# hiimmuc/SpeakerVerification

Measured on AMD Instinct MI355X. Metric: embeddings/sec (2 s @16 kHz), higher is better.
Workload: dtype bf16

## Files before the change

### speakerverification_amd/csrc/api.hip

```cpp
#include <algorithm>
#include <cstdlib>
#include <cstring>

#include "handle.h"

using namespace svhip;

namespace svhip {
RaggedCheckFn ecapa_ragged_check, rawnet2_ragged_check, rawnet3_ragged_check, conformer_ragged_check, titanet_ragged_check, resnetse_ragged_check;
RaggedEmbedFn ecapa_embed_ragged, rawnet2_embed_ragged, rawnet3_embed_ragged, conformer_embed_ragged, titanet_embed_ragged, resnetse_embed_ragged;
}

namespace {

thread_local std::string g_create_error;

enum DevOptParse { OPT_NO_ENV, OPT_SET, OPT_IS1, OPT_NUM };
struct DevOptRow { const char* name; int svhip_handle::DevOpts::*field; const char* env; DevOptParse parse; int dflt; };
#define SV_OPT(name, env, parse, dflt) {#name, &svhip_handle::DevOpts::name, env, parse, dflt}
const DevOptRow kDevOpts[] = {
    SV_OPT(layer_labels, "SVHIP_LAYER_LABELS", OPT_SET, 0),
    SV_OPT(x3_keep_f32, "SVHIP_X3_KEEP_F32", OPT_SET, 0),
    SV_OPT(r2_big, "SVHIP_R2_BIG", OPT_IS1, 0),
    SV_OPT(asp_v1, "SVHIP_ASP_V1", OPT_IS1, 0),
// ... 7 lines not shown
    SV_OPT(asnorm_norefit, nullptr, OPT_NO_ENV, 0),
    SV_OPT(rn_sinc_full, "SVHIP_RN_SINC_FULL", OPT_IS1, 0),
    SV_OPT(fbank32, "SVHIP_FBANK32", OPT_IS1, 0),
    SV_OPT(fbank_unfused, "SVHIP_FBANK_UNFUSED", OPT_IS1, 0),
    SV_OPT(pw3_cus, "SVHIP_PW3_CUS", OPT_NUM, -1),
    SV_OPT(pw3_tail_off, "SVHIP_PW3_TAIL_OFF", OPT_IS1, 0),
    SV_OPT(cv_off, "SVHIP_CV_OFF", OPT_IS1, 0),
    SV_OPT(n128_off, "SVHIP_N128_OFF", OPT_IS1, 0),
    SV_OPT(rn_pool_off, "SVHIP_RN_POOL_OFF", OPT_IS1, 0),
    SV_OPT(rn_step_off, "SVHIP_RN_STEP_OFF", OPT_IS1, 0),
    SV_OPT(rn_sinc_f32, "SVHIP_RN_SINC_F32", OPT_IS1, 0),
    SV_OPT(rn_tail_big, "SVHIP_RN_TAIL_BIG", OPT_IS1, 0),
    SV_OPT(r2_slices, "SVHIP_R2_SLICES", OPT_NUM, -1),
    SV_OPT(rn_conv_unfused, "SVHIP_RN_CONV_UNFUSED", OPT_IS1, 0),
    SV_OPT(rn_keep, "SVHIP_RN_KEEP", OPT_IS1, 0),
};
#undef SV_OPT

int none_check(const svhip_config& c, const char*& err) {
    if (c.compute == SVHIP_F16) { err = "SVHIP_F16 is RawNet2's 16-bit mode (ECAPA's is SVHIP_BF16)"; return SVHIP_ERR_UNSUPPORTED; }
    return SVHIP_OK;
}
int fbank_then_features(svhip_handle* h, const float* d_wav, int B);

const ModelOps kModels[] = {
    {SVHIP_MODEL_ECAPA,        ecapa_check,     ecapa_spec,     ecapa_finalize,     ecapa_alloc,     ecapa_embed_wave,    ecapa_forward,     ecapa_stage,     2,
     nullptr, ecapa_ragged_check, ecapa_embed_ragged},
    {SVHIP_MODEL_RAWNET2,      rawnet2_check,   rawnet2_spec,   rawnet2_finalize,   rawnet2_alloc,   rawnet2_forward,     nullptr,           rawnet2_stage,   4},
    {SVHIP_MODEL_RAWNET2_CONV, rawnet2_check,   rawnet2_spec,   rawnet2_finalize,   rawnet2_alloc,   rawnet2_forward,     nullptr,           rawnet2_stage,   4,
     nullptr, rawnet2_ragged_check, rawnet2_embed_ragged},
// ... 12 lines not shown
const ModelOps* model_ops(int model) {
    for (const ModelOps& m : kModels)
        if (m.model == model) return &m;
    return nullptr;
}

WeightSpec model_spec(const svhip_handle* h) {
    WeightSpec spec;
    if (const ModelOps* m = model_ops(h->cfg.model); m->spec) m->spec(h->cfg, spec);
    return spec;
}

int fbank_then_features(svhip_handle* h, const float* d_wav, int B) {
    int rc;
    if ((rc = run(h, "fbank", 0, [&]() { return launch_fbank(h->fb, d_wav, B, h->cfg.samples, h->T, h->d_feat, h->stream); }))) return rc;
    h->feat_is_stale = false;
    return model_ops(h->cfg.model)->embed_feat(h, h->d_feat, B);
}

}

namespace svhip {

hipEvent_t prof_event(svhip_handle* h) {
    if (!h->ev_free.empty()) { hipEvent_t e = h->ev_free.back(); h->ev_free.pop_back(); return e; }
    hipEvent_t e = nullptr;
    (void)hipEventCreate(&e);
    return e;
}

void prof_collect(svhip_handle* h) {
// ... 335 lines not shown
int svhip_embed_features(svhip_handle* h, const float* feat, int32_t B, int32_t T, float* emb_out, int32_t flags) {
    int rc = check_ready(h, B);
    if (rc) return rc;
    if (!feat || !emb_out) SV_FAIL(h, SVHIP_ERR_INVALID, "null pointer");
    const ModelOps* m = model_ops(h->cfg.model);
    if (!m->embed_feat) SV_FAIL(h, SVHIP_ERR_UNSUPPORTED, "embed_features needs a spectral model (ECAPA, TitaNet, Conformer, ResNetSE)");
    if (T != h->T) SV_FAIL(h, SVHIP_ERR_INVALID, "T=%d but the handle was created for T=%d frames", T, h->T);
    if ((flags & SVHIP_ASYNC) && (flags & (SVHIP_IN_DEVICE | SVHIP_OUT_DEVICE)) != (SVHIP_IN_DEVICE | SVHIP_OUT_DEVICE))
        SV_FAIL(h, SVHIP_ERR_INVALID, "SVHIP_ASYNC needs device pointers");
    SV_HIP(h, hipSetDevice(h->cfg.device));
    const float* d_in = feat;
    if (!(flags & SVHIP_IN_DEVICE)) {
        SV_HIP(h, hipMemcpyAsync(h->d_feat, feat, (size_t)B * h->cfg.n_mels * T * 4, hipMemcpyHostToDevice, h->stream));
        d_in = h->d_feat;
    }
    h->feat_is_stale = false;
    if ((rc = m->embed_feat(h, d_in, B))) return rc;
    if ((rc = emit_embeddings(h, B, emb_out, flags))) return rc;
    return finish(h, flags);
}

int svhip_embed_wave(svhip_handle* h, const float* wav, int32_t B, int32_t L, float* emb_out, int32_t flags) {
    int rc = check_ready(h, B);
    if (rc) return rc;
    if (!wav || !emb_out) SV_FAIL(h, SVHIP_ERR_INVALID, "null pointer");
    if (L != h->cfg.samples) SV_FAIL(h, SVHIP_ERR_INVALID, "L=%d but the handle was created for %d samples", L, h->cfg.samples);
    if ((flags & SVHIP_ASYNC) && (flags & (SVHIP_IN_DEVICE | SVHIP_OUT_DEVICE)) != (SVHIP_IN_DEVICE | SVHIP_OUT_DEVICE))
        SV_FAIL(h, SVHIP_ERR_INVALID, "SVHIP_ASYNC needs device pointers");
    const ModelOps* m = model_ops(h->cfg.model);
    if (!m->embed_wave) SV_FAIL(h, SVHIP_ERR_UNSUPPORTED, "model %d has no forward path in this build", h->cfg.model);
    SV_HIP(h, hipSetDevice(h->cfg.device));
// ... 139 lines not shown
    if (!rc && tmp) e = hipMemcpyAsync(wav_out, d_out, (size_t)B * L * 4, hipMemcpyDeviceToHost, h->stream);
    if (tmp || !(flags & SVHIP_ASYNC)) { const hipError_t e2 = hipStreamSynchronize(h->stream); if (e == hipSuccess) e = e2; }
    if (tmp) (void)hipFree(tmp);
    if (rc) return rc;
    SV_HIP(h, e);
    return SVHIP_OK;
}

int svhip_get_stage(svhip_handle* h, const char* name, float* out, int64_t* count) {
    if (!h || !name || !count) return SVHIP_ERR_INVALID;
    if (h->lastB <= 0) SV_FAIL(h, SVHIP_ERR_STATE, "no forward has run yet");
    const int B = h->lastB;
    const size_t rag_in = h->rag_levels ? (size_t)h->rag_rows[0] : 0;
    StageView v{nullptr, rag_in ? rag_in : (size_t)B * h->T, 0, 0, !h->bf16};
    const std::string n(name);
    if (n == "input" && h->X_in) { v.src = h->X_in; v.cols = v.ld = h->cfg.n_mels; }
    else if (n == "mel") {
        if (h->feat_is_stale) SV_FAIL(h, SVHIP_ERR_STATE, "stage mel: the last forward ran the fused front-end, which never forms the mel power "
                                      "tensor (option fbank_unfused = 1 keeps the separate kernels)");
        v.src = h->d_feat; v.rows = (size_t)B * h->cfg.n_mels; v.cols = v.ld = h->T; v.f32 = true;
        if (rag_in) { v.rows = 1; v.cols = v.ld = rag_in * h->cfg.n_mels; }
    }
    else {
        const ModelOps* m = model_ops(h->cfg.model);
        if (!m->stage) return unknown_stage(h, n);
        if (int rc = m->stage(h, n, out != nullptr, v)) return rc;
    }
    const size_t rows = v.rows, cols = v.cols;
    *count = (int64_t)(rows * cols);
    if (!out) return SVHIP_OK;
    SV_HIP(h, hipStreamSynchronize(h->stream));
// ... 63 lines not shown
```

### speakerverification_amd/csrc/api_ecapa.hip

```cpp
#include <algorithm>

#include "handle.h"

namespace svhip {

namespace {

struct EcapaState : ModelState {
    ConvLayer blocks0, mfa, asp_tdnn, asp_conv;
    ConvLayer tdnn1[3], tdnn2[3], res2[3][7];
    LinearLayer se1[3], se2[3], asp_ctx, fc;
    float* se2T[3] = {};
    void *se1_bf[3] = {}, *se2T_bf[3] = {};
    float *aspbn_scale = nullptr, *aspbn_shift = nullptr;

    bool xin_ready = false;
    bool x0_is_s32 = false;
    bool cat_f32_stale = false;
    bool h2_is_s32 = false;
    bool h1_split = false;
    void* cat_s32 = nullptr;
    void* h2_s32 = nullptr;
    void* u_s32[2] = {};
    void* X0 = nullptr;
    void *H1 = nullptr, *H2 = nullptr, *H3 = nullptr;
    void* CAT = nullptr;
    void* MFA = nullptr;
    void* ATT = nullptr;
    float* LOGITS = nullptr;
    float *d_mean = nullptr, *d_s1 = nullptr, *d_s2 = nullptr, *d_gstats = nullptr, *d_ctx = nullptr;
    float *d_pool_raw = nullptr, *d_pool_bn = nullptr;
// ... 117 lines not shown
    if ((rc = dev_alloc(h, &s.d_gstats, B * 2 * C3))) return rc;
    if ((rc = dev_alloc(h, &s.d_ctx, B * 128))) return rc;
    h->lin_part_per_utt = (size_t)((2 * C3 + 383) / 384) * (size_t)std::max(128, c.embed_dim);
    if ((rc = dev_alloc(h, &h->d_lin_part, B * h->lin_part_per_utt))) return rc;
    if ((rc = dev_alloc(h, &s.d_pool_raw, B * 2 * C3))) return rc;
    if ((rc = dev_alloc(h, &s.d_pool_bn, B * 2 * C3))) return rc;
    if (h->x3 && (rc = dev_alloc(h, reinterpret_cast<char**>(&h->s32_buf), M * C3 * 4 + 256))) return rc;
    if (h->x3 && C % 32 == 0 && (rc = dev_alloc(h, reinterpret_cast<char**>(&s.cat_s32), M * C3 * 4 + 256))) return rc;
    if (h->x3 && (C == 512 || C == 1024)) {
        if ((rc = dev_alloc(h, reinterpret_cast<char**>(&s.h2_s32), M * C * 4 + 256))) return rc;
        for (int i = 0; i < 2; ++i) if ((rc = dev_alloc(h, reinterpret_cast<char**>(&s.u_s32[i]), M * (C / 8) * 4 + 256))) return rc;
    }
    h->colsum_region = (int64_t)((M + 255) / 256 + 2) * 16 * C3;
    if ((rc = dev_alloc(h, &h->d_colsum, (size_t)4 * h->colsum_region))) return rc;
    return SVHIP_OK;
}

static int ecapa_forward_part(svhip_handle* h, const float* d_feat_all, int b0, int B) {
    auto& s = S(h);
    const svhip_config& c = h->cfg;
    const int T = h->T, M = B * T, C = c.channels, C3 = 3 * C, C8 = C / 8, e = h->esz;
    const bool bf = h->bf16;
    hipStream_t st = h->cur;
    const size_t r0 = (size_t)b0 * T;
    const float* d_feat = d_feat_all + (size_t)b0 * c.n_mels * T;
    void* X_in = off(h->X_in, r0 * c.n_mels, e);
    void* X0 = off(s.X0, r0 * C, e);
    void* H1 = off(s.H1, r0 * C, e);
    void* H2 = off(s.H2, r0 * C, e);
    void* H3 = off(s.H3, r0 * C, e);
// ... 36 lines not shown
    if (!s.xin_ready && (rc = run(h, "prologue", 0, [&]() {
             return launch_prologue(d_feat, X_in, bf, B, c.n_mels, T, c.log_input, h->in_w, h->in_b, d_pstats, st,
                                    h->x3 ? h->d_status : nullptr, h->host_flag_dev, (b0_cv && xscale) ? 3.0e38f : 65504.0f);
         }))) return rc;
    if (b0_cv) {
        const ConvLayer& L = s.blocks0;
        if (xscale && (rc = run(h, "in_scale", 0, [&]() {
                 return launch_in_scale(static_cast<const float*>(X_in), (int64_t)M * c.n_mels, reinterpret_cast<uint32_t*>(xscale + 4), xscale, st, L.cv_wscale);
             }))) return rc;
        if ((rc = run(h, "split_s32", 0, [&]() { return launch_split_s32(static_cast<const float*>(X_in), c.n_mels, h->s32_buf, M, L.cv_cin, st, L.cv_cin, c.n_mels, xscale); }))) return rc;
        if ((rc = run(h, "gemm_pw3cv", (double)M * L.flops_per_row, [&]() { return launch_gemm_pw3cv(q0, st); }))) return rc;
        b0_done = true;
        x0_s32 = q0.y_s32 != 0;
    }
    if (!b0_done) {
        GemmParams p = conv_params(h, s.blocks0, X_in, c.n_mels, X0, C, M, T);
        p.act1 = ACT_GELU;
        if ((rc = conv_gemm(h, s.blocks0, p))) return rc;
    }
    s.x0_is_s32 = x0_s32;
    const void* xin = x0_s32 ? nullptr : X0;
    int ldin = C;
    const void* xin32 = x0_s32 ? X0 : nullptr;
    int ldin32 = C;
    for (int i = 0; i < 3; ++i) {
        char* h2s = s.h2_s32 ? static_cast<char*>(s.h2_s32) + r0 * C * 4 : nullptr;
        char* us[2] = {s.u_s32[0] ? static_cast<char*>(s.u_s32[0]) + r0 * C8 * 4 : nullptr, s.u_s32[1] ? static_cast<char*>(s.u_s32[1]) + r0 * C8 * 4 : nullptr};
        auto step_params = [&](int j) {
            const ConvLayer& L = s.res2[i][j - 1];
            GemmParams q = conv_params(h, L, us[(j - 1) & 1], C8, h2s + (size_t)j * C8 * 4, C, M, T);
            q.W = L.Ws32; q.Wrows = L.N; q.x3 = 2; q.act1 = ACT_RELU;
            if (j < 7) { q.R = static_cast<const float*>(H1) + (size_t)(j + 1) * C8; q.ldr = C; q.Y2 = us[j & 1]; q.lda2 = C8; }
// ... 113 lines not shown
         }))) return rc;
    return SVHIP_OK;
}

int ecapa_forward(svhip_handle* h, const float* d_feat, int B) {
    S(h).cat_f32_stale = false;
    const bool two = h->lanes == 2 && B >= 64 && !h->x3;
    return forward_lanes(h, ecapa_forward_part, d_feat, B, two ? 2 : 1, (B / 2 + 3) & ~3);
}

int ecapa_embed_wave(svhip_handle* h, const float* d_wav, int B) {
    auto& s = S(h);
    const int L = h->cfg.samples, T = h->T;
    const bool fused = h->bf16 && !h->in_w && h->d_logmel && !h->opt.fbank_unfused && !h->opt.fbank32 && fbank_fused_supported(h->fb, L);
    int rc;
    if (fused) {
        if ((rc = run(h, "fbank_fused", 0, [&]() {
                 return launch_fbank_fused(h->fb, d_wav, B, L, T, h->cfg.log_input, h->d_logmel, h->d_fpart, h->X_in, h->stream);
             }))) return rc;
    } else if ((rc = run(h, "fbank", 0, [&]() { return launch_fbank(h->fb, d_wav, B, L, T, h->d_feat, h->stream); }))) return rc;
    s.xin_ready = fused;
    h->feat_is_stale = fused;
    rc = ecapa_forward(h, h->d_feat, B);
    s.xin_ready = false;
    return rc;
}

int ecapa_ragged_check(const svhip_config& c, const int32_t* lengths, int n, bool is_wave, std::string& err) {
    return rag_mel_check(c, lengths, n, is_wave, err, true, "hop_length / max_batch / samples", 5, " (block 3 reflect-pads 4 frames on each side)");
}

static void ecapa_rag_frames(const svhip_config& c, int64_t len, bool is_wave, int T[RAG_LEVELS]) { T[0] = (int)mel_frames(c, len, is_wave); }
static const RagRule kEcapaRag = {1, ecapa_rag_frames, true};

static int ecapa_forward_ragged(svhip_handle* h, const RagPack& pk) {
    auto& s = S(h);
    const svhip_config& c = h->cfg;
    const int C = c.channels, C3 = 3 * C, C8 = C / 8, e = h->esz;
    const bool bf = h->bf16;
// ... 120 lines not shown
```

### speakerverification_amd/csrc/api_gemm.hip

```cpp
#include "handle.h"

namespace svhip {

static const void* zero_page_for(const svhip_handle* h, const void* A) {
    const char* a = static_cast<const char*>(A);
    for (const TailedBuf& b : h->tailed)
        if (a >= b.base && a < b.base + b.bytes) return b.base + b.bytes;
    return h->d_zero;
}

GemmParams conv_params(const svhip_handle* h, const ConvLayer& L, const void* A, int lda, void* Y, int ldy, int M, int T) {
    GemmParams p;
    p.A = A; p.lda = lda; p.Y = Y; p.ldy = ldy;
    p.W = L.W; p.Wrows = L.Np; p.bias = L.bias; p.scale = L.scale; p.shift = L.shift;
    p.M = M; p.N = L.N; p.K = L.K; p.Kp = L.Kp; p.T = T; p.taps = L.taps; p.dil = L.dil; p.cin = L.cin;
    p.num_cu = h->num_cu; p.pw3_cus = h->opt.pw3_cus; p.tail_split = h->opt.pw3_tail_off ? 0 : 1;
    p.zeros = h->d_zeros; p.ones = h->d_ones; p.f16 = h->f16 ? 1 : 0;
    p.cv_off = h->opt.cv_off; p.n128_off = h->opt.n128_off;
    return p;
}

GemmPlan conv_plan(const svhip_handle* h, const ConvLayer& L, GemmParams p, const void* A_s32, int lda_s32) {
    GemmPlan g;
    p.zero_page = zero_page_for(h, p.A);
    const int M = p.M;
    const bool bf = h->bf16;
    g.flops = (double)M * (L.flops_per_row + 2.0 * L.N * p.K3);
    if (h->x3 && L.Ws32 && h->s32_buf && !p.A2 && !p.bias_utt && !p.out_f32 && !p.R) {
        GemmParams q = p;
        q.A = A_s32 ? A_s32 : h->s32_buf; q.lda = A_s32 ? lda_s32 : L.K; q.W = L.Ws32; q.x3 = 2;
        if (!gemm_pw3x3_supported(q)) q.side_a = q.side_b = nullptr, q.side_c = 0;
        if (!gemm_pw3x3_supported(q) && q.colsum) q.colsum = nullptr;
        if (gemm_pw3x3_supported(q)) {
// ... 40 lines not shown
```

### speakerverification_amd/csrc/api_ragged.hip

```cpp
#include <algorithm>
#include <cstdarg>

#include "handle.h"

namespace svhip {

int refuse(std::string& err, int code, const char* fmt, ...) {
    char b[512];
    va_list ap;
    va_start(ap, fmt);
    vsnprintf(b, sizeof(b), fmt, ap);
    va_end(ap);
    err = b;
    return code;
}

int rag_rows_fit(std::string& err, int i, int64_t rows, int64_t cap, const char* frames_name) {
    if (rows <= cap) return SVHIP_OK;
    return refuse(err, SVHIP_ERR_INVALID, "utterance %d: the pack reaches %lld frames, over the handle's capacity of max_batch * %s = %lld rows", i,
                  (long long)rows, frames_name, (long long)cap);
}

int rag_mel_check(const svhip_config& c, const int32_t* lengths, int n, bool is_wave, std::string& err, bool cfg_extra_ok, const char* cfg_names,
                  int min_frames, const char* why, RagUttRule* more, int64_t bound, int row_unit) {
// ... 38 lines not shown
    return SVHIP_OK;
}

RagTables::~RagTables() {
    for (auto& sl : slot) {
        if (sl.host) (void)hipHostFree(sl.host);
        if (sl.done) (void)hipEventDestroy(sl.done);
    }
}

static int rag_mel_input(svhip_handle* h, RagTables& rag, const float* in, bool in_host, bool is_wave, const int64_t* in_off, const int32_t* lengths,
                  int n, const int* mel0, int64_t* feat_off, const float** d_feat) {
    const svhip_config& c = h->cfg;
    int rc;
    *d_feat = h->d_feat;
    h->feat_is_stale = false;
    if (is_wave) {
        int64_t pos = 0;
        for (int u = 0; u < n; ++u) {
            const int L = lengths[u], T = mel0[u + 1] - mel0[u];
            const float* w = in + in_off[u];
            if (in_host) {
                SV_HIP(h, hipMemcpyAsync(rag.wav + pos, w, (size_t)L * 4, hipMemcpyHostToDevice, h->stream));
                w = rag.wav + pos;
                pos += L;
            }
            float* mel = h->d_feat + (size_t)mel0[u] * c.n_mels;
            if ((rc = run(h, "fbank", 0, [&]() { return launch_fbank(h->fb, w, 1, L, T, mel, h->stream); }))) return rc;
            feat_off[u] = (int64_t)mel0[u] * c.n_mels;
        }
    } else if (in_host) {
// ... 78 lines not shown
```

### speakerverification_amd/csrc/fbank.hip

```cpp
#include <stdlib.h>

#include "common.h"
#include "kernels.h"

namespace svhip {

namespace {

constexpr int FB_FRAMES = 32;
constexpr int FB_THREADS = 192;
constexpr int FB_PT_STRIDE = 289;
constexpr int FB_PAIRS_PER_WAVE = 3;

template <bool SPLIT>
__global__ __launch_bounds__(FB_THREADS) void fbank_kernel(FbankTables tb, const float* __restrict__ wav,
                                                           int L, int T, float* __restrict__ mel) {
    extern __shared__ __attribute__((aligned(16))) char smem[];
    const int ns = (FB_FRAMES - 1) * tb.hop + tb.win_length;
    const int ns_pad = ((ns + 15) & ~15) + 16;
    float* ys = reinterpret_cast<float*>(smem);
    float* pt = ys + ns_pad;
    float* melw = pt + FB_FRAMES * FB_PT_STRIDE;

    const int b = blockIdx.y;
// ... 655 lines not shown

bool fbank_fused_supported(const FbankTables& tb, int L) {
    return tb.sym_hi && tb.sym_lo && tb.n_fft == 512 && tb.win_length == 200 && tb.hop == 80 && tb.lpad == 156 && tb.mel_max_bin < 256 &&
           tb.n_mels % 4 == 0 && 32 * tb.n_mels <= 5 * FF_THREADS && tb.n_pairs >= 8 && L >= tb.n_fft && fbank_fused_lds(tb) <= 80 * 1024 &&
           (size_t)(32 * FF_PT_STRIDE + 32 * (tb.n_mels + 1)) * 4 <= (size_t)4 * FF_PLANE;
}

hipError_t launch_fbank_fused(const FbankTables& tb, const float* wav, int B, int L, int T, int log_input, float* logmel, float* partial,
                              void* out, hipStream_t stream) {
    if (!fbank_fused_supported(tb, L) || B <= 0) return hipErrorInvalidValue;
    const size_t lds = fbank_fused_lds(tb);
    static DeviceOnce attr;
    if (hipError_t e = set_max_dynamic_lds(attr, reinterpret_cast<const void*>(fbank_fused_kernel), 80 * 1024)) return e;
    const int ntiles = (T + FF_FRAMES - 1) / FF_FRAMES;
    hipLaunchKernelGGL(fbank_fused_kernel, dim3(ntiles, B), dim3(FF_THREADS), lds, stream, tb, wav, L, T, log_input, logmel, partial);
    hipLaunchKernelGGL(fbank_norm_kernel<bf16_t>, dim3((T + 63) / 64, B), dim3(256), 0, stream, logmel, partial, reinterpret_cast<bf16_t*>(out), T,
                       tb.n_mels, ntiles, log_input);
    return hipGetLastError();
}

hipError_t launch_prologue(const float* feat, void* out, bool out_bf16, int B, int n_mels, int T, int log_input,
                           const float* in_w, const float* in_b, float* stats, hipStream_t stream, uint32_t* status, uint32_t* host_flag, float limit) {
    const int rows = B * n_mels;
    hipLaunchKernelGGL(prologue_stats_kernel, dim3((rows + 3) / 4), dim3(256), 0, stream, feat, stats, rows, T,
                       log_input, in_w != nullptr ? 1 : 0);
    dim3 grid((T + 31) / 32, B);
    const size_t lds = (size_t)n_mels * 33 * sizeof(float);
    if (out_bf16)
        hipLaunchKernelGGL(prologue_apply_kernel<bf16_t>, grid, dim3(256), lds, stream, feat, stats,
                           reinterpret_cast<bf16_t*>(out), n_mels, T, log_input, in_w, in_b, status, host_flag, limit);
// ... 8 lines not shown
```

### speakerverification_amd/csrc/gemm_pw2.hip

```cpp
#include "common.h"
#include "kernels.h"
#include "gemm_epi.h"

namespace svhip {

namespace {

typedef __attribute__((address_space(3))) void lds_void;
typedef __attribute__((address_space(1))) const void gbl_void;

constexpr int QBM = 256, QBN = 256;
constexpr int HT = 16384;
constexpr int PW2_LDS = 8 * HT;
#ifdef QGROUP_M_OVERRIDE
constexpr int QGROUP_M = QGROUP_M_OVERRIDE;
#else
constexpr int QGROUP_M = 12;
#endif

#ifdef SVHIP_GEMM_DEBUG
constexpr bool DBG2 = true;
#else
constexpr bool DBG2 = false;
#endif
// ... 364 lines not shown
        if (p.lda3 <= 0 || p.lda % p.lda3 != 0 || ((p.lda / p.lda3) & (p.lda / p.lda3 - 1)) != 0 || p.lda3 % 8 != 0 || p.K3 > p.lda3) return false;
        if (reinterpret_cast<uintptr_t>(p.A3) & 15) return false;
    }
    if (p.taps > 1) {
        if (!p.zero_page || p.cin % 8 != 0 || p.taps * p.cin != p.K || p.T <= 0 || p.M % p.T != 0) return false;
        if (p.pad_mode == PAD_REFLECT && (p.taps / 2) * p.dil >= p.T) return false;
        if (p.Kp >= 65536 || p.cin > 1024) return false;
        return true;
    }
    return p.K == p.Kp;
}

hipError_t launch_gemm_pw2(const GemmParams& p, hipStream_t stream) {
    if (!gemm_pw2_supported(p, true) || p.M <= 0 || p.Wrows < p.N) return hipErrorInvalidValue;
    const bool conv = p.taps > 1;
    if (p.A3) return launch_inst<EPI_NONE, 2>(p, stream);
    if (p.act2 == ACT_LRELU03) return conv ? launch_inst<EPI_BN_LRELU03, 1>(p, stream) : launch_inst<EPI_BN_LRELU03, 0>(p, stream);
    switch (p.act1) {
        case ACT_NONE: return conv ? launch_inst<EPI_NONE, 1>(p, stream) : launch_inst<EPI_NONE, 0>(p, stream);
        case ACT_RELU: return conv ? launch_inst<EPI_RELU, 1>(p, stream) : launch_inst<EPI_RELU, 0>(p, stream);
        case ACT_GELU: return conv ? launch_inst<EPI_GELU, 1>(p, stream) : launch_inst<EPI_GELU, 0>(p, stream);
        case ACT_LRELU03: return conv ? launch_inst<EPI_LRELU03, 1>(p, stream) : launch_inst<EPI_LRELU03, 0>(p, stream);
        default: return hipErrorInvalidValue;
    }
}

}
```

### speakerverification_amd/csrc/handle.h

```cpp
#pragma once
#include "../../include/svhip.h"

#include <hip/hip_runtime.h>

#include <cstdio>
#include <initializer_list>
#include <map>
#include <memory>
#include <string>
#include <vector>

#include "common.h"
#include "kernels.h"

namespace svhip {

struct HostTensor {
    std::vector<float> data;
    std::vector<int64_t> shape;
    int64_t numel() const { int64_t n = 1; for (auto s : shape) n *= s; return n; }
};

struct ConvLayer {
    int N = 0, K = 0, Kp = 0, Np = 0, taps = 1, dil = 1, cin = 0;
// ... 47 lines not shown
        int score_tiled;
        int asnorm_norefit;
        int rn_sinc_full;
        int fbank32;
        int fbank_unfused;
        int pw3_cus;
        int pw3_tail_off;
        int cv_off;
        int n128_off;
        int rn_pool_off;
        int rn_step_off;
        int rn_sinc_f32;
        int rn_tail_big;
        int r2_slices;
        int rn_conv_unfused;
        int rn_keep;
    } opt;
    bool bf16 = false;
    bool f16 = false;
    int dt = svhip::DT_F32;
    bool x3 = false;
    bool finalized = false;
    std::string err;
    std::map<std::string, svhip::HostTensor> host_w;
    std::vector<void*> allocs;

    int T = 0;
    int esz = 4;

    svhip::FbankTables fb;
    int num_cu = 256;

    std::unique_ptr<svhip::ModelState> model;

    float* d_wav = nullptr;
    float* d_feat = nullptr;
    float* d_pstats = nullptr;
    float* d_xscale = nullptr;
    float* d_logmel = nullptr;
    float* d_fpart = nullptr;
    bool feat_is_stale = false;
    float* d_zero = nullptr;
    float *d_ones = nullptr, *d_zeros = nullptr;
    float* d_emb = nullptr;
    int lastB = 0;
    int64_t rag_rows[svhip::RAG_LEVELS] = {};
    int rag_levels = 0;
    void* X_in = nullptr;
    float *in_w = nullptr, *in_b = nullptr;
    float* d_colsum = nullptr;
    int64_t colsum_region = 0;
    float* d_lin_part = nullptr;
    size_t lin_part_per_utt = 0;
    void* s32_buf = nullptr;
    std::vector<svhip::TailedBuf> tailed;
    uint32_t* d_status = nullptr;
// ... 188 lines not shown
```

### speakerverification_amd/csrc/kernels.h

```cpp
#pragma once
#include <hip/hip_runtime.h>
#include <stdint.h>

#include <atomic>

#include "common.h"

namespace svhip {

struct DeviceOnce {
    std::atomic<uint64_t> mask{0};
    bool done(int dev) const { return dev >= 0 && dev < 64 && ((mask.load(std::memory_order_acquire) >> dev) & 1u); }
    void mark(int dev) { if (dev >= 0 && dev < 64) mask.fetch_or(1ull << dev, std::memory_order_release); }
};
inline hipError_t set_max_dynamic_lds(DeviceOnce& once, const void* fn, int bytes) {
    int dev = -1;
    hipError_t e = hipGetDevice(&dev);
    if (e != hipSuccess) return e;
    if (once.done(dev)) return hipSuccess;
    e = hipFuncSetAttribute(fn, hipFuncAttributeMaxDynamicSharedMemorySize, bytes);
    if (e == hipSuccess) once.mark(dev);
    return e;
}

// ... 13 lines not shown
    const float* ones = nullptr;
    const void* zero_page = nullptr;
    void* Y2 = nullptr;
    const void* R = nullptr;
    int ldr = 0;
    const void* A3 = nullptr;
    int lda3 = 0, K3 = 0;
    int y_s32 = 0;
    void* side_a = nullptr;
    void* side_b = nullptr;
    int side_lda = 0, side_ldb = 0, side_c = 0;
    int num_cu = 256;
    int n128_off = 0;
    int cv_off = 0;
    int pw3_cus = -1;
    const float* in_scale = nullptr;
    int tail_split = 1;
    void* ts = nullptr;
    int M = 0, N = 0, K = 0, Kp = 0;
    int lda = 0, lda2 = 0, ldy = 0, ld_bu = 0;
    int T = 1;
    uint32_t t_magic = 0;
    int taps = 1, dil = 1, cin = 0, pad_mode = 0;
    int act1 = 0, act2 = 0;
    int out_f32 = 0;
    int f16 = 0;
    int x3 = 0;
    int debug = 0;
    int Wrows = 0;
    const int* seg_off = nullptr;
// ... 6 lines not shown

constexpr int GEMM_BM = 128;
constexpr int GEMM_BN = 128;
constexpr int GEMM_BK_BYTES = 128;

inline int gemm_bk(bool bf16) { return bf16 ? 64 : 32; }
inline int round_up(int x, int m) { return (x + m - 1) / m * m; }

hipError_t launch_gemm(const GemmParams& p, bool bf16, hipStream_t stream);
enum GemmRoute : int { ROUTE_PW2 = 0, ROUTE_PW = 1, ROUTE_PW_NARROW = 2, ROUTE_GENERIC = 3, ROUTE_PW3 = 4, ROUTE_PW3CV = 5, ROUTE_N128 = 6 };
GemmRoute gemm_route(const GemmParams& p, bool bf16);
bool gemm_pw_supported(const GemmParams& p, bool bf16);
hipError_t launch_gemm_pw(const GemmParams& p, bool bf16, hipStream_t stream, bool narrow = false);
bool gemm_pw2_supported(const GemmParams& p, bool bf16);
hipError_t launch_gemm_pw2(const GemmParams& p, hipStream_t stream);
bool gemm_pw3_supported(const GemmParams& p, bool bf16);
hipError_t launch_gemm_pw3(const GemmParams& p, hipStream_t stream);
int pw3_grid_cap(const GemmParams& p);
bool gemm_pw3x3_supported(const GemmParams& p);
hipError_t launch_gemm_pw3x3(const GemmParams& p, hipStream_t stream);
bool r2_step_supported(const GemmParams& p);
hipError_t launch_r2_step(const GemmParams& p, hipStream_t stream);
bool rn_step_supported(const GemmParams& p, int mode);
hipError_t launch_rn_step(const GemmParams& p, int mode, hipStream_t stream);
bool gemm_pw3cv_supported(const GemmParams& p);
hipError_t launch_gemm_pw3cv(const GemmParams& p, hipStream_t stream);
bool gemm_n128_supported(const GemmParams& p);
hipError_t launch_gemm_n128(const GemmParams& p, hipStream_t stream);
bool gemm_pw3cv16_supported(const GemmParams& p);
hipError_t launch_gemm_pw3cv16(const GemmParams& p, hipStream_t stream);
// ... 50 lines not shown
    const int* mel_start = nullptr;
    const int* mel_len = nullptr;
    const int* mel_off = nullptr;
    int n_fft = 512, win_length = 200, hop = 80, n_mels = 80, n_bins = 257, lpad = 156;
    int n_pairs = 9;
    int n_q = 25;
    int mel_max_bin = 256;
    int force32 = 0;
    float preemph = 0.97f;
};
hipError_t launch_fbank(const FbankTables& tb, const float* wav, int B, int L, int T, float* mel, hipStream_t stream);

bool fbank_fused_supported(const FbankTables& tb, int L);
hipError_t launch_fbank_fused(const FbankTables& tb, const float* wav, int B, int L, int T, int log_input, float* logmel, float* partial,
                              void* out, hipStream_t stream);

hipError_t launch_prologue(const float* feat, void* out, bool out_bf16, int B, int n_mels, int T,
                           int log_input, const float* in_w, const float* in_b, float* stats, hipStream_t stream,
                           uint32_t* status = nullptr, uint32_t* host_flag = nullptr, float limit = 3.0e38f);

hipError_t launch_colmean(const void* X, int dt, int ldx, int B, int T, int C, float* mean, hipStream_t stream,
                          float* scratch = nullptr, int scratch_slices = 0);
hipError_t launch_colstats(const void* X, bool bf16, int ldx, int B, int T, int C, float* stats, float eps, hipStream_t stream);
size_t rowvec_linear_scratch_bytes(int B, int N, int K, bool short_rows = false);
hipError_t launch_rowvec_linear(const float* in, int ld_in, const float* W, const float* bias, float* out, int ld_out,
                                int B, int N, int K, int act, hipStream_t stream, float* part = nullptr, bool short_rows = false);
hipError_t launch_emb_out(const float* src, float* dst, int n, uint32_t* status, uint32_t* host_flag, hipStream_t stream);
hipError_t launch_se_mlp(const float* mean, const float* part, int T, const void* W1, const float* b1, const void* W2T,
                         const float* b2, float* s, bool w_bf16, int B, int C, int H, hipStream_t stream, int row_groups = 8);
hipError_t launch_se_apply(const void* h, int ldh, const float* s, const void* x, int ldx, void* out, int ldo,
// ... 258 lines not shown
```

Before: 59430.

## Fuse fbank mean-normalization into a weight-stationary blocks.0 conv kernel

Adds a new weight-stationary conv kernel for ECAPA's first 5-tap conv (80 input channels), which keeps the weights in registers and double-buffers reflect-padded input tiles in LDS. When the fused front-end is active, the kernel reads fp32 log-mel rows and per-utterance partial sums directly, subtracts the mean and casts to bf16 on the fly. This skips the separate fbank_norm kernel and the bf16 X_in round trip. The normalized input is now formed lazily only if a stage dump asks for it. The cost is a larger specialized code path with a heavier LDS footprint, and new state flags to track staleness.

```diff
diff --git a/speakerverification_amd/csrc/api.hip b/speakerverification_amd/csrc/api.hip
--- a/speakerverification_amd/csrc/api.hip
+++ b/speakerverification_amd/csrc/api.hip
@@ -45,6 +45,7 @@
     SV_OPT(r2_slices, "SVHIP_R2_SLICES", OPT_NUM, -1),
     SV_OPT(rn_conv_unfused, "SVHIP_RN_CONV_UNFUSED", OPT_IS1, 0),
     SV_OPT(rn_keep, "SVHIP_RN_KEEP", OPT_IS1, 0),
+    SV_OPT(b0_ws_off, "SVHIP_B0_WS_OFF", OPT_IS1, 0),
 };
 #undef SV_OPT
 
@@ -87,7 +88,7 @@
 int fbank_then_features(svhip_handle* h, const float* d_wav, int B) {
     int rc;
     if ((rc = run(h, "fbank", 0, [&]() { return launch_fbank(h->fb, d_wav, B, h->cfg.samples, h->T, h->d_feat, h->stream); }))) return rc;
-    h->feat_is_stale = false;
+    h->feat_is_stale = h->xin_is_stale = false;
     return model_ops(h->cfg.model)->embed_feat(h, h->d_feat, B);
 }
 
@@ -453,7 +454,7 @@
         SV_HIP(h, hipMemcpyAsync(h->d_feat, feat, (size_t)B * h->cfg.n_mels * T * 4, hipMemcpyHostToDevice, h->stream));
         d_in = h->d_feat;
     }
-    h->feat_is_stale = false;
+    h->feat_is_stale = h->xin_is_stale = false;
     if ((rc = m->embed_feat(h, d_in, B))) return rc;
     if ((rc = emit_embeddings(h, B, emb_out, flags))) return rc;
     return finish(h, flags);
@@ -623,7 +624,13 @@
     const size_t rag_in = h->rag_levels ? (size_t)h->rag_rows[0] : 0;
     StageView v{nullptr, rag_in ? rag_in : (size_t)B * h->T, 0, 0, !h->bf16};
     const std::string n(name);
-    if (n == "input" && h->X_in) { v.src = h->X_in; v.cols = v.ld = h->cfg.n_mels; }
+    if (n == "input" && h->X_in) {
+        v.src = h->X_in; v.cols = v.ld = h->cfg.n_mels;
+        if (h->xin_is_stale && out) {
+            SV_HIP(h, launch_fbank_norm(h->fb, h->d_logmel, h->d_fpart, h->X_in, B, h->T, h->cfg.log_input, h->stream));
+            h->xin_is_stale = false;
+        }
+    }
     else if (n == "mel") {
         if (h->feat_is_stale) SV_FAIL(h, SVHIP_ERR_STATE, "stage mel: the last forward ran the fused front-end, which never forms the mel power "
                                       "tensor (option fbank_unfused = 1 keeps the separate kernels)");
diff --git a/speakerverification_amd/csrc/api_ecapa.hip b/speakerverification_amd/csrc/api_ecapa.hip
--- a/speakerverification_amd/csrc/api_ecapa.hip
+++ b/speakerverification_amd/csrc/api_ecapa.hip
@@ -15,6 +15,7 @@
     float *aspbn_scale = nullptr, *aspbn_shift = nullptr;
 
     bool xin_ready = false;
+    bool xin_ws = false;
     bool x0_is_s32 = false;
     bool cat_f32_stale = false;
     bool h2_is_s32 = false;
@@ -162,6 +163,24 @@
     h->colsum_region = (int64_t)((M + 255) / 256 + 2) * 16 * C3;
     if ((rc = dev_alloc(h, &h->d_colsum, (size_t)4 * h->colsum_region))) return rc;
     return SVHIP_OK;
+}
+
+static GemmParams blocks0_params(svhip_handle* h, int b0, int B, bool from_logmel) {
+    auto& s = S(h);
+    const svhip_config& c = h->cfg;
+    const size_t r0 = (size_t)b0 * h->T;
+    GemmParams p = conv_params(h, s.blocks0, off(h->X_in, r0 * c.n_mels, h->esz), c.n_mels, off(s.X0, r0 * c.channels, h->esz), c.channels, B * h->T, h->T);
+    p.act1 = ACT_GELU;
+    if (from_logmel) {
+        p.ws_logmel = h->d_logmel + r0 * c.n_mels;
+        p.ws_fpart = h->d_fpart + (size_t)b0 * ((h->T + 63) / 64) * c.n_mels;
+        p.ws_sub_mean = c.log_input;
+    }
+    return p;
+}
+static bool blocks0_takes_ws(svhip_handle* h, const GemmParams& p) {
+    const GemmPlan g = conv_plan(h, S(h).blocks0, p);
+    return !g.x3 && g.route == ROUTE_PW2 && conv_ws_supported(g.q);
 }
 
 static int ecapa_forward_part(svhip_handle* h, const float* d_feat_all, int b0, int B) {
@@ -228,8 +247,9 @@
         x0_s32 = q0.y_s32 != 0;
     }
     if (!b0_done) {
-        GemmParams p = conv_params(h, s.blocks0, X_in, c.n_mels, X0, C, M, T);
-        p.act1 = ACT_GELU;
+        GemmParams p = blocks0_params(h, b0, B, s.xin_ws);
+        if (s.xin_ws && !blocks0_takes_ws(h, p))
+            SV_FAIL(h, SVHIP_ERR_STATE, "blocks.0 M%d: the front-end left only its fp32 rows and the kernel that reads them does not take this shape", M);
         if ((rc = conv_gemm(h, s.blocks0, p))) return rc;
     }
     s.x0_is_s32 = x0_s32;
@@ -373,15 +393,23 @@
     const int L = h->cfg.samples, T = h->T;
     const bool fused = h->bf16 && !h->in_w && h->d_logmel && !h->opt.fbank_unfused && !h->opt.fbank32 && fbank_fused_supported(h->fb, L);
     int rc;
+    bool ws = fused && !h->opt.b0_ws_off;
+    if (ws) {
+        const bool two = h->lanes == 2 && B >= 64;
+        const int per = two ? (B / 2 + 3) & ~3 : B;
+        for (int b0 = 0; b0 < B && ws; b0 += per) ws = blocks0_takes_ws(h, blocks0_params(h, b0, std::min(per, B - b0), true));
+    }
     if (fused) {
         if ((rc = run(h, "fbank_fused", 0, [&]() {
-                 return launch_fbank_fused(h->fb, d_wav, B, L, T, h->cfg.log_input, h->d_logmel, h->d_fpart, h->X_in, h->stream);
+                 return launch_fbank_fused(h->fb, d_wav, B, L, T, h->cfg.log_input, h->d_logmel, h->d_fpart, ws ? nullptr : h->X_in, h->stream);
              }))) return rc;
     } else if ((rc = run(h, "fbank", 0, [&]() { return launch_fbank(h->fb, d_wav, B, L, T, h->d_feat, h->stream); }))) return rc;
     s.xin_ready = fused;
+    s.xin_ws = ws;
     h->feat_is_stale = fused;
     rc = ecapa_forward(h, h->d_feat, B);
-    s.xin_ready = false;
+    s.xin_ready = s.xin_ws = false;
+    h->xin_is_stale = ws;
     return rc;
 }
 
diff --git a/speakerverification_amd/csrc/api_gemm.hip b/speakerverification_amd/csrc/api_gemm.hip
--- a/speakerverification_amd/csrc/api_gemm.hip
+++ b/speakerverification_amd/csrc/api_gemm.hip
@@ -16,7 +16,7 @@
     p.M = M; p.N = L.N; p.K = L.K; p.Kp = L.Kp; p.T = T; p.taps = L.taps; p.dil = L.dil; p.cin = L.cin;
     p.num_cu = h->num_cu; p.pw3_cus = h->opt.pw3_cus; p.tail_split = h->opt.pw3_tail_off ? 0 : 1;
     p.zeros = h->d_zeros; p.ones = h->d_ones; p.f16 = h->f16 ? 1 : 0;
-    p.cv_off = h->opt.cv_off; p.n128_off = h->opt.n128_off;
+    p.cv_off = h->opt.cv_off; p.n128_off = h->opt.n128_off; p.ws_off = h->opt.b0_ws_off;
     return p;
 }
 
diff --git a/speakerverification_amd/csrc/api_ragged.hip b/speakerverification_amd/csrc/api_ragged.hip
--- a/speakerverification_amd/csrc/api_ragged.hip
+++ b/speakerverification_amd/csrc/api_ragged.hip
@@ -76,7 +76,7 @@
     const svhip_config& c = h->cfg;
     int rc;
     *d_feat = h->d_feat;
-    h->feat_is_stale = false;
+    h->feat_is_stale = h->xin_is_stale = false;
     if (is_wave) {
         int64_t pos = 0;
         for (int u = 0; u < n; ++u) {
diff --git a/speakerverification_amd/csrc/conv_ws.hip b/speakerverification_amd/csrc/conv_ws.hip
--- /dev/null
+++ b/speakerverification_amd/csrc/conv_ws.hip
@@ -0,0 +1,278 @@
+#include <algorithm>
+
+#include "common.h"
+#include "kernels.h"
+#include "gemm_epi.h"
+
+namespace svhip {
+
+namespace {
+
+constexpr int WS_BM = 64;
+constexpr int WS_BN = 128;
+constexpr int WS_NCK = 13;
+constexpr int WS_TMIN = 32;
+constexpr int WS_SEGS = 3;
+constexpr int WS_MAXHALO = 2;
+constexpr int WS_CIN = 80;
+constexpr int WS_ROWS = WS_BM + 2 * WS_MAXHALO * WS_SEGS;
+constexpr int WS_OSTRIDE = 80;
+constexpr int WS_OPATCH = WS_BM * WS_OSTRIDE;
+constexpr int WS_THREADS = 256;
+constexpr int WS_NU = 16;
+#ifdef WS_ABL
+constexpr int ABL = WS_ABL;
+#else
+constexpr int ABL = 0;
+#endif
+
+struct WsGeom {
+    int rowb;
+    int ximg;
+    int mean_off;
+    int out_off;
+    int total;
+};
+__host__ __device__ constexpr WsGeom ws_geom(int cin) {
+    WsGeom g{};
+    g.rowb = cin * 2;
+    g.ximg = ((WS_ROWS + 1) * g.rowb + 63) & ~63;
+    g.mean_off = 2 * g.ximg;
+    g.out_off = g.mean_off + ((WS_NU * cin * 4 + 63) & ~63);
+    g.total = g.out_off + 4 * WS_OPATCH;
+    return g;
+}
+
+template <int MODE>
+__global__ __launch_bounds__(WS_THREADS, 2) void conv_ws_kernel(GemmParams p, int nslice, int G, int ntile) {
+    extern __shared__ __attribute__((aligned(16))) char smem[];
+    constexpr WsGeom g = ws_geom(WS_CIN);
+    constexpr int cin = WS_CIN;
+    const int tid = threadIdx.x, lane = tid & 63;
+    const int wave = __builtin_amdgcn_readfirstlane(tid >> 6);
+    const int r16 = lane & 15, q4 = lane >> 4;
+
+    const int id = blockIdx.x;
+    const int slice = (id >> 3) % nslice;
+    const int j = (id & 7) + 8 * ((id >> 3) / nslice);
+    if (j >= G) return;
+    const int tile_lo = (int)((int64_t)j * ntile / G), tile_hi = (int)((int64_t)(j + 1) * ntile / G);
+    if (tile_lo >= tile_hi) return;
+
+    const int T = p.T, halo = p.taps >> 1, TP = T + 2 * halo, B = p.M / T;
+    constexpr int cpr = cin >> 3;
+    constexpr int nchunk = WS_ROWS * cpr;
+    const int ntf = (T + 63) / 64;
+
+    const int nw0 = slice * WS_BN + wave * 32;
+    bf16x8 wf[2][WS_NCK];
+#pragma unroll
+    for (int jj = 0; jj < 2; ++jj) {
+        const char* wr = reinterpret_cast<const char*>(p.W) + ((int64_t)(nw0 + jj * 16 + r16) * p.Kp + q4 * 8) * 2;
+#pragma unroll
+        for (int c = 0; c < WS_NCK; ++c) wf[jj][c] = *reinterpret_cast<const bf16x8*>(wr + c * 64);
+    }
+    f32x4 b4[2], sc4[2], sh4[2];
+#pragma unroll
+    for (int jj = 0; jj < 2; ++jj) {
+        const int n = nw0 + jj * 16 + 4 * q4;
+        b4[jj] = p.bias ? *reinterpret_cast<const f32x4*>(p.bias + n) : f32x4{0.f, 0.f, 0.f, 0.f};
+        sc4[jj] = f32x4{1.f, 1.f, 1.f, 1.f}; sh4[jj] = f32x4{0.f, 0.f, 0.f, 0.f};
+        if (p.scale) { sc4[jj] = *reinterpret_cast<const f32x4*>(p.scale + n); sh4[jj] = *reinterpret_cast<const f32x4*>(p.shift + n); }
+    }
+
+    char* const ximg = smem;
+    float* const means = reinterpret_cast<float*>(smem + g.mean_off);
+    char* const opatch = smem + g.out_off + wave * WS_OPATCH;
+    const int ua = (tile_lo * WS_BM) / T;
+
+    constexpr int NIT = (nchunk + WS_THREADS - 1) / WS_THREADS;
+    u32x4 st[MODE == 0 ? NIT : 2 * NIT];
+    int st_r[NIT], st_cg[NIT];
+#pragma unroll
+    for (int it = 0; it < NIT; ++it) {
+        const int cc = min(it * WS_THREADS + tid, nchunk - 1);
+        st_r[it] = cc / cpr; st_cg[it] = cc - st_r[it] * cpr;
+    }
+    auto src_row = [&](int tile, int r, int& s) -> int64_t {
+        const int m0 = tile * WS_BM, u0 = m0 / T, t0 = m0 - u0 * T;
+        const int q = r + t0;
+        s = (q >= TP ? 1 : 0) + (q >= 2 * TP ? 1 : 0);
+        const int tr = reflect_idx(q - s * TP - halo, T);
+        return (int64_t)min(u0 + s, B - 1) * T + tr;
+    };
+    auto load_tile = [&](int tile) {
+#pragma unroll
+        for (int it = 0; it < NIT; ++it) {
+            int s;
+            const int64_t row = src_row(tile, st_r[it], s);
+            if (MODE == 0) {
+                st[it] = *reinterpret_cast<const u32x4*>(reinterpret_cast<const char*>(p.A) + (row * p.lda + st_cg[it] * 8) * 2);
+            } else {
+                const u32x4* src = reinterpret_cast<const u32x4*>(p.ws_logmel + row * cin + st_cg[it] * 8);
+                st[2 * it] = src[0]; st[2 * it + 1] = src[1];
+            }
+        }
+    };
+    auto store_tile = [&](int tile, char* img) {
+#pragma unroll
+        for (int it = 0; it < NIT; ++it) {
+            {
+                const int r = st_r[it], cg = st_cg[it];
+                u32x4 v;
+                if (MODE == 0) {
+                    v = st[it];
+                } else {
+                    const int m0 = tile * WS_BM, u0 = m0 / T, t0 = m0 - u0 * T, q = r + t0;
+                    const int s = (q >= TP ? 1 : 0) + (q >= 2 * TP ? 1 : 0);
+                    const float* mean = means + (min(u0 + s, B - 1) - ua) * cin + cg * 8;
+                    const f32x4 m_lo = *reinterpret_cast<const f32x4*>(mean);
+                    const f32x4 m_hi = *reinterpret_cast<const f32x4*>(mean + 4);
+                    const f32x4 a = __builtin_bit_cast(f32x4, st[2 * it]), b = __builtin_bit_cast(f32x4, st[2 * it + 1]);
+                    bf16x8 y;
+#pragma unroll
+                    for (int e = 0; e < 4; ++e) { y[e] = from_f32<bf16_t>(a[e] - m_lo[e]); y[4 + e] = from_f32<bf16_t>(b[e] - m_hi[e]); }
+                    v = __builtin_bit_cast(u32x4, y);
+                }
+                *reinterpret_cast<u32x4*>(img + r * g.rowb + cg * 16) = v;
+            }
+        }
+    };
+    load_tile(tile_lo);
+    if (MODE == 1) {
+        const int ub = min(B - 1, ((tile_hi - 1) * WS_BM) / T + WS_SEGS - 1);
+        const float rcin = 1.0f / (float)cin;
+        for (int idx = tid; idx < (ub - ua + 1) * cin; idx += WS_THREADS) {
+            const int du = (int)(((float)idx + 0.5f) * rcin), ch = idx - du * cin;
+            const float* src = p.ws_fpart + (int64_t)(ua + du) * ntf * cin + ch;
+            float sum = 0.0f;
+            for (int k0 = 0; k0 < ntf; k0 += 8) {
+                float v[8];
+#pragma unroll
+                for (int kk = 0; kk < 8; ++kk) v[kk] = src[min(k0 + kk, ntf - 1) * cin];
+#pragma unroll
+                for (int kk = 0; kk < 8; ++kk) sum = k0 + kk < ntf ? sum + v[kk] : sum;
+            }
+            means[idx] = p.ws_sub_mean ? sum / (float)T : 0.0f;
+        }
+        __syncthreads();
+    }
+    store_tile(tile_lo, ximg);
+    __syncthreads();
+
+    const int kmask = p.K - (WS_NCK - 1) * 32 - q4 * 8;
+    char* const Yb = reinterpret_cast<char*>(p.Y);
+    for (int tile = tile_lo; tile < tile_hi; ++tile) {
+        const int k = tile - tile_lo;
+        const char* xb = ximg + (k & 1) * g.ximg;
+        const int next = min(tile + 1, tile_hi - 1);
+        load_tile(next);
+        __builtin_amdgcn_sched_barrier(0);
+
+        const int m0 = tile * WS_BM, t0 = m0 - (m0 / T) * T;
+        int xo[4];
+#pragma unroll
+        for (int i = 0; i < 4; ++i) {
+            const int q = i * 16 + r16 + t0;
+            const int s = (q >= T ? 1 : 0) + (q >= 2 * T ? 1 : 0);
+            xo[i] = (i * 16 + r16 + 2 * halo * s) * g.rowb + q4 * 16;
+        }
+        f32x4 acc[4][2];
+#pragma unroll
+        for (int i = 0; i < 4; ++i) { acc[i][0] = b4[0]; acc[i][1] = b4[1]; }
+#pragma unroll
+        for (int c = 0; c < WS_NCK; ++c) {
+            bf16x8 xf[4];
+#pragma unroll
+            for (int i = 0; i < 4; ++i) {
+                xf[i] = *reinterpret_cast<const bf16x8*>(xb + xo[i] + c * 64);
+                if (c == WS_NCK - 1) {
+                    u32x4 z = __builtin_bit_cast(u32x4, xf[i]);
+                    z = kmask > 0 ? z : u32x4{0u, 0u, 0u, 0u};
+                    xf[i] = __builtin_bit_cast(bf16x8, z);
+                }
+            }
+#pragma unroll
+            for (int i = 0; i < 4; ++i)
+#pragma unroll
+                for (int jj = 0; jj < 2; ++jj)
+                    if (!(ABL & 1)) acc[i][jj] = Half16<bf16_t>::mfma16(wf[jj][c], xf[i], acc[i][jj]);
+        }
+
+        store_tile(next, ximg + ((k + 1) & 1) * g.ximg);
+
+#pragma unroll
+        for (int i = 0; i < 4; ++i)
+#pragma unroll
+            for (int jj = 0; jj < 2; ++jj) {
+                float v[4];
+                if (ABL & 4) { v[0] = acc[i][jj][0]; v[1] = acc[i][jj][1]; v[2] = acc[i][jj][2]; v[3] = acc[i][jj][3]; }
+                else act4<EPI_GELU>(v, acc[i][jj], sc4[jj], sh4[jj]);
+                typedef bf16_t bf16x4 __attribute__((ext_vector_type(4)));
+                const bf16x4 o = {static_cast<bf16_t>(v[0]), static_cast<bf16_t>(v[1]), static_cast<bf16_t>(v[2]), static_cast<bf16_t>(v[3])};
+                *reinterpret_cast<bf16x4*>(opatch + (i * 16 + r16) * WS_OSTRIDE + (jj * 16 + 4 * q4) * 2) = o;
+            }
+        __builtin_amdgcn_fence(__ATOMIC_RELEASE, "wavefront");
+        __builtin_amdgcn_wave_barrier();
+        __builtin_amdgcn_fence(__ATOMIC_ACQUIRE, "wavefront");
+#pragma unroll
+        for (int it = 0; it < 4; ++it) {
+            const int row = it * 16 + (lane >> 2), ch = lane & 3;
+            const u32x4 d = *reinterpret_cast<const u32x4*>(opatch + row * WS_OSTRIDE + ch * 16);
+            const int m = m0 + row;
+            if (m < p.M && !(ABL & 8)) *reinterpret_cast<u32x4*>(Yb + ((int64_t)m * p.ldy + nw0 + ch * 8) * 2) = d;
+        }
+        __syncthreads();
+    }
+}
+
+}
+
+static int ws_groups(const GemmParams& p) {
+    const int nslice = p.N / WS_BN, ntile = (p.M + WS_BM - 1) / WS_BM;
+    return std::max(1, std::min(ntile, 2 * p.num_cu / nslice));
+}
+static int ws_tiles_per_wg(const GemmParams& p) {
+    const int ntile = (p.M + WS_BM - 1) / WS_BM, G = ws_groups(p);
+    return (ntile + G - 1) / G;
+}
+
+bool conv_ws_supported(const GemmParams& p) {
+    if (p.ws_off || p.f16 || p.out_f32 || p.bias_utt || p.A2 || p.A3 || p.R || p.colsum || p.seg_off || p.rag_utt || p.x3) return false;
+    if (p.act1 != ACT_GELU || p.act2 != ACT_NONE || p.pad_mode != PAD_REFLECT || p.dil != 1) return false;
+    if (p.taps != 5 || p.cin != WS_CIN || p.taps * p.cin != p.K) return false;
+    if (p.K <= (WS_NCK - 1) * 32 || p.K > WS_NCK * 32 || p.Kp < WS_NCK * 32 || p.Kp % 8 != 0) return false;
+    if (p.T < WS_TMIN || p.M <= 0 || p.M % p.T != 0) return false;
+    if (p.N <= 0 || p.N % WS_BN != 0 || p.Wrows < p.N || p.ldy % 8 != 0 || p.ldy < p.N) return false;
+    if ((reinterpret_cast<uintptr_t>(p.W) | reinterpret_cast<uintptr_t>(p.Y)) & 15) return false;
+    if (p.bias && (reinterpret_cast<uintptr_t>(p.bias) & 15)) return false;
+    if (p.scale && (!p.shift || ((reinterpret_cast<uintptr_t>(p.scale) | reinterpret_cast<uintptr_t>(p.shift)) & 15))) return false;
+    if (p.ws_logmel) {
+        if (!p.ws_fpart || ((reinterpret_cast<uintptr_t>(p.ws_logmel) | reinterpret_cast<uintptr_t>(p.ws_fpart)) & 15)) return false;
+        if ((ws_tiles_per_wg(p) - 1) * WS_BM / p.T + WS_SEGS + 1 > WS_NU) return false;
+    } else if (!p.A || p.lda % 8 != 0 || p.lda < p.cin || (reinterpret_cast<uintptr_t>(p.A) & 15)) {
+        return false;
+    }
+    return true;
+}
+
+hipError_t launch_conv_ws(const GemmParams& p, hipStream_t stream) {
+    if (!conv_ws_supported(p)) return hipErrorInvalidValue;
+    const int nslice = p.N / WS_BN, ntile = (p.M + WS_BM - 1) / WS_BM;
+    const int G = ws_groups(p);
+    const int Gp = (G + 7) & ~7;
+    constexpr int lds = ws_geom(WS_CIN).total;
+    static_assert(lds <= 64 * 1024, "two workgroups per CU");
+    if (p.ws_logmel) {
+        static DeviceOnce attr;
+        if (hipError_t e = set_max_dynamic_lds(attr, reinterpret_cast<const void*>(conv_ws_kernel<1>), lds)) return e;
+        hipLaunchKernelGGL(conv_ws_kernel<1>, dim3(Gp * nslice), dim3(WS_THREADS), lds, stream, p, nslice, G, ntile);
+    } else {
+        static DeviceOnce attr;
+        if (hipError_t e = set_max_dynamic_lds(attr, reinterpret_cast<const void*>(conv_ws_kernel<0>), lds)) return e;
+        hipLaunchKernelGGL(conv_ws_kernel<0>, dim3(Gp * nslice), dim3(WS_THREADS), lds, stream, p, nslice, G, ntile);
+    }
+    return hipGetLastError();
+}
+
+}
diff --git a/speakerverification_amd/csrc/fbank.hip b/speakerverification_amd/csrc/fbank.hip
--- a/speakerverification_amd/csrc/fbank.hip
+++ b/speakerverification_amd/csrc/fbank.hip
@@ -693,6 +693,13 @@
     if (hipError_t e = set_max_dynamic_lds(attr, reinterpret_cast<const void*>(fbank_fused_kernel), 80 * 1024)) return e;
     const int ntiles = (T + FF_FRAMES - 1) / FF_FRAMES;
     hipLaunchKernelGGL(fbank_fused_kernel, dim3(ntiles, B), dim3(FF_THREADS), lds, stream, tb, wav, L, T, log_input, logmel, partial);
+    if (hipError_t e = hipGetLastError()) return e;
+    return out ? launch_fbank_norm(tb, logmel, partial, out, B, T, log_input, stream) : hipSuccess;
+}
+
+hipError_t launch_fbank_norm(const FbankTables& tb, const float* logmel, const float* partial, void* out, int B, int T, int log_input,
+                             hipStream_t stream) {
+    const int ntiles = (T + FF_FRAMES - 1) / FF_FRAMES;
     hipLaunchKernelGGL(fbank_norm_kernel<bf16_t>, dim3((T + 63) / 64, B), dim3(256), 0, stream, logmel, partial, reinterpret_cast<bf16_t*>(out), T,
                        tb.n_mels, ntiles, log_input);
     return hipGetLastError();
diff --git a/speakerverification_amd/csrc/gemm_pw2.hip b/speakerverification_amd/csrc/gemm_pw2.hip
--- a/speakerverification_amd/csrc/gemm_pw2.hip
+++ b/speakerverification_amd/csrc/gemm_pw2.hip
@@ -402,6 +402,8 @@
 hipError_t launch_gemm_pw2(const GemmParams& p, hipStream_t stream) {
     if (!gemm_pw2_supported(p, true) || p.M <= 0 || p.Wrows < p.N) return hipErrorInvalidValue;
     const bool conv = p.taps > 1;
+    if (conv && conv_ws_supported(p)) return launch_conv_ws(p, stream);
+    if (p.ws_logmel) return hipErrorInvalidValue;
     if (p.A3) return launch_inst<EPI_NONE, 2>(p, stream);
     if (p.act2 == ACT_LRELU03) return conv ? launch_inst<EPI_BN_LRELU03, 1>(p, stream) : launch_inst<EPI_BN_LRELU03, 0>(p, stream);
     switch (p.act1) {
diff --git a/speakerverification_amd/csrc/handle.h b/speakerverification_amd/csrc/handle.h
--- a/speakerverification_amd/csrc/handle.h
+++ b/speakerverification_amd/csrc/handle.h
@@ -85,6 +85,7 @@
         int rn_tail_big;
         int r2_slices;
         int rn_conv_unfused;
+        int b0_ws_off;
         int rn_keep;
     } opt;
     bool bf16 = false;
@@ -111,6 +112,7 @@
     float* d_logmel = nullptr;
     float* d_fpart = nullptr;
     bool feat_is_stale = false;
+    bool xin_is_stale = false;
     float* d_zero = nullptr;
     float *d_ones = nullptr, *d_zeros = nullptr;
     float* d_emb = nullptr;
diff --git a/speakerverification_amd/csrc/kernels.h b/speakerverification_amd/csrc/kernels.h
--- a/speakerverification_amd/csrc/kernels.h
+++ b/speakerverification_amd/csrc/kernels.h
@@ -51,6 +51,10 @@
     int n128_off = 0;
     int cv_off = 0;
     int pw3_cus = -1;
+    int ws_off = 0;
+    const float* ws_logmel = nullptr;
+    const float* ws_fpart = nullptr;
+    int ws_sub_mean = 0;
     const float* in_scale = nullptr;
     int tail_split = 1;
     void* ts = nullptr;
@@ -87,6 +91,8 @@
 hipError_t launch_gemm_pw(const GemmParams& p, bool bf16, hipStream_t stream, bool narrow = false);
 bool gemm_pw2_supported(const GemmParams& p, bool bf16);
 hipError_t launch_gemm_pw2(const GemmParams& p, hipStream_t stream);
+bool conv_ws_supported(const GemmParams& p);
+hipError_t launch_conv_ws(const GemmParams& p, hipStream_t stream);
 bool gemm_pw3_supported(const GemmParams& p, bool bf16);
 hipError_t launch_gemm_pw3(const GemmParams& p, hipStream_t stream);
 int pw3_grid_cap(const GemmParams& p);
@@ -167,6 +173,8 @@
 bool fbank_fused_supported(const FbankTables& tb, int L);
 hipError_t launch_fbank_fused(const FbankTables& tb, const float* wav, int B, int L, int T, int log_input, float* logmel, float* partial,
                               void* out, hipStream_t stream);
+hipError_t launch_fbank_norm(const FbankTables& tb, const float* logmel, const float* partial, void* out, int B, int T, int log_input,
+                             hipStream_t stream);
 
 hipError_t launch_prologue(const float* feat, void* out, bool out_bf16, int B, int n_mels, int T,
                            int log_input, const float* in_w, const float* in_b, float* stats, hipStream_t stream,
```

Result: no change. 59890, median of 6 (+0.8%).
